# 0xC0000054/avif-format

Measured on NVIDIA H100. Metric: Gpixels/s, higher is better.
Workload: dtype f32

## Files before the change

### avif-format_b200/csrc/kernels_fast_flat.cu

```cuda
#include "kernels_fast_common.cuh"
#include "launch_keys.h"
#include "table_staging.cuh"
#include "../../include/avifgpu.h"

namespace avifgpu
{

using namespace avifpix;
using namespace fastenc;
using namespace staging;
using avifmath::LibmTables;

namespace
{

constexpr int kFlatThreads = kFlatWarps * 32;
constexpr int kRowSegmentBytes = kTilePixels * 12;
static_assert(kFlatStageBytesPerWarp == 2 * kRowSegmentBytes, "a warp's staging buffer holds both rows of its tile");
constexpr int kRowSegmentWords = kRowSegmentBytes / 4;
constexpr int kTableBarrierSlot = kFlatSharedBarriers / 8 - 1;
static_assert(kFlatWarps <= kTableBarrierSlot, "the warps' barriers and the table's share kFlatSharedBarriers");

struct FlatSchedule
{
    int32_t tilesX, tileRows, warpCount;
    int32_t segments, items;
    int32_t segmentRows, longSegments;
    int32_t lastColumnBytes;
    int32_t unpairedTileRow;
};

__device__ __forceinline__ bool ElectOne()
{
    uint32_t elected;
    asm volatile("{ .reg .pred p; elect.sync _|p, 0xffffffff; selp.u32 %0, 1, 0, p; }" : "=r"(elected));
    return elected != 0;
}

constexpr int kTableTwoLevel = 1;
constexpr int kTableCompact = 2;
constexpr int kTableCompact14 = 3;

template <int CURVE, int XS, int YS, int TABLE, int INTERLEAVED, int DEST>
__device__ __forceinline__ void EncodeRgbF32FlatBody(const FastEncodeParams& p, const FlatSchedule& schedule)
{
    constexpr bool kCompact = TABLE != kTableTwoLevel;
    constexpr int kCompactShift = TABLE == kTableCompact14 ? 14 : 0;
    extern __shared__ __align__(128) uint8_t sharedBytes[];
    uint64_t* libmStorage = reinterpret_cast<uint64_t*>(sharedBytes);
    uint64_t* barriers = reinterpret_cast<uint64_t*>(sharedBytes + kSharedLibm);
    uint8_t* stageAll = sharedBytes + kSharedLibm + kFlatSharedBarriers;
    uint32_t* compactEntries = reinterpret_cast<uint32_t*>(sharedBytes + FlatFixedBytes());
    const uint32_t* firstBits = compactEntries + ((p.table.flatCount + 3) & ~3);
    uint2* octaves = reinterpret_cast<uint2*>(sharedBytes + FlatFixedBytes());
    uint32_t* bucketWords = reinterpret_cast<uint32_t*>(sharedBytes + FlatFixedBytes() + kFlatOctaveBytes);

    const int lane = threadIdx.x & 31;
    const int warpInBlock = __shfl_sync(0xffffffffu, static_cast<int>(threadIdx.x >> 5), 0);
    const uint32_t barrier = SharedAddress(barriers + warpInBlock);
    uint32_t* stage = reinterpret_cast<uint32_t*>(stageAll + warpInBlock * kFlatStageBytesPerWarp);
    const uint32_t stageAddress = SharedAddress(stage);
    const uint32_t* myStage = stage + lane * 12;

    const int tilesX = schedule.tilesX;
    const int warpCount = schedule.warpCount;
    const int firstItem = warpInBlock * static_cast<int>(gridDim.x) + static_cast<int>(blockIdx.x);
    constexpr int kChromaRowsPerTile = YS ? 1 : 2;
    constexpr int kChromaPairs = SourceInterleaved(DEST) ? 2 : 1;
    constexpr int kChromaTileBytes = (XS ? kTilePixels : 2 * kTilePixels) * kChromaPairs;

    auto itemRows = [&](int item, int& column, int& rowBegin, int& rowEnd)
    {
        const int segment = item / tilesX;
        column = item - segment * tilesX;
        rowBegin = segment * schedule.segmentRows + min(segment, schedule.longSegments);
        rowEnd = rowBegin + schedule.segmentRows + (segment < schedule.longSegments ? 1 : 0);
    };
    auto fetchTile = [&](int row, uint32_t bytes, int64_t offset)
    {
        const bool second = row != schedule.unpairedTileRow;
        const uint8_t* source = p.rows + offset;
        BarrierExpect(barrier, second ? 2u * bytes : bytes);
        BulkCopyToShared(stageAddress, source, bytes, barrier);
        if (second)
        {
            BulkCopyToShared(stageAddress + kRowSegmentBytes, source + p.rowStride, bytes, barrier);
        }
    };
    auto columnBytes = [&](int column) { return column == tilesX - 1 ? static_cast<uint32_t>(schedule.lastColumnBytes) : static_cast<uint32_t>(kRowSegmentBytes); };
    auto sourceOffsetOf = [&](int row, int column) { return static_cast<int64_t>(row) * 2 * p.rowStride + static_cast<int64_t>(column) * kRowSegmentBytes; };

    if (kCompact && threadIdx.x == 0)
    {
        BeginTableImageCopy(p.table, compactEntries, barriers + kTableBarrierSlot);
    }
    if (ElectOne())
    {
        BarrierInit(barrier, 1);
        BarrierInitFence();
        if (firstItem < schedule.items)
        {
            int column, rowBegin, rowEnd;
            itemRows(firstItem, column, rowBegin, rowEnd);
            if (rowBegin < rowEnd)
            {
                fetchTile(rowBegin, columnBytes(column), sourceOffsetOf(rowBegin, column));
            }
        }
    }

    const LibmTables t = avifmath::StageLibmTables(libmStorage, threadIdx.x, blockDim.x);
    if (!kCompact)
    {
        for (int i = threadIdx.x; i < 256; i += blockDim.x)
        {
            octaves[i] = p.table.octaves[i];
        }
        for (int i = threadIdx.x; i < p.table.bucketCount; i += blockDim.x)
        {
            bucketWords[i] = p.table.buckets[i];
        }
    }
    __syncthreads();
    if (kCompact)
    {
        WaitTableImage(barriers + kTableBarrierSlot);
    }

    const uint32_t flatShift = p.table.flatShift;
    const int32_t negativeLow = -static_cast<int32_t>(p.table.flatLow);
    const int32_t span = static_cast<int32_t>(p.table.flatHigh - p.table.flatLow);
    const uint32_t bandStrideLog2 = p.table.bandStrideLog2;
    const uint32_t* __restrict__ bandBits = p.table.bandBits;
    const uint32_t compactTopShift = 32u - flatShift;
    const uint32_t compactCodeMask = p.table.compactCodeMask;
    const uint32_t compactMagic = p.table.compactMagic;
    uint32_t parity = 0;

#pragma unroll 1
    for (int item = firstItem; item < schedule.items; item += warpCount)
    {
        int column, rowBegin, rowEnd;
        itemRows(item, column, rowBegin, rowEnd);
        if (item != firstItem && rowBegin < rowEnd && ElectOne())
        {
            fetchTile(rowBegin, columnBytes(column), sourceOffsetOf(rowBegin, column));
        }
        const uint32_t tileBytes = columnBytes(column);
        const bool laneActive = column * kTilePixels + lane * 4 < p.width;
        int64_t sourceOffset = sourceOffsetOf(rowBegin, column);
        uint8_t* yPointer = p.planeY + static_cast<int64_t>(rowBegin) * 2 * p.strideY +
                            (INTERLEAVED ? static_cast<int64_t>(column) * (6 * kTilePixels) + lane * 24 : static_cast<int64_t>(column) * (2 * kTilePixels) + lane * 8);
        uint8_t* cbPointer = p.planeCb + static_cast<int64_t>(rowBegin) * kChromaRowsPerTile * p.strideCb + static_cast<int64_t>(column) * kChromaTileBytes + lane * (XS ? 4 : 8) * kChromaPairs;
        uint8_t* crPointer = p.planeCr + static_cast<int64_t>(rowBegin) * kChromaRowsPerTile * p.strideCr + static_cast<int64_t>(column) * kChromaTileBytes + lane * (XS ? 4 : 8);

#pragma unroll 1
    for (int tileRow = rowBegin; tileRow < rowEnd; ++tileRow)
    {
        const bool secondRow = tileRow != schedule.unpairedTileRow;
        sourceOffset += 2 * p.rowStride;

        BarrierWait(barrier, parity);
        parity ^= 1u;

        float codeF[kValuesPerLane];
        uint32_t bandMask = 0;
        int32_t largest = 0;
#pragma unroll
        for (int q = 0; q < 6; ++q)
        {
            const uint4 w = *reinterpret_cast<const uint4*>(myStage + (q / 3) * kRowSegmentWords + (q % 3) * 4);
            const uint32_t bits[4] = { w.x, w.y, w.z, w.w };
#pragma unroll
            for (int e = 0; e < 4; ++e)
            {
                const int j = 4 * q + e;
                bool inBand;
                if (kCompact)
                {
                    uint32_t entry;
                    codeF[j] = LookupCurveCompact<kCompactShift>(bits[e], compactEntries, flatShift, negativeLow, span, compactTopShift, compactCodeMask,
                                                                 compactMagic, inBand, entry);
                }
                else
                {
                    codeF[j] = CodeToFloat(LookupCurveCode(bits[e], octaves, bucketWords, inBand));
                }
                asm("{ .reg .pred p; setp.ne.u32 p, %1, 0; @p or.b32 %0, %0, %2; }" : "+r"(bandMask) : "r"(static_cast<uint32_t>(inBand)), "r"(1u << j));
            }
            if (kCompact)
            {
                largest = max(largest, __vimax3_s32(static_cast<int32_t>(w.x), static_cast<int32_t>(w.y), static_cast<int32_t>(w.z)));
                largest = max(largest, static_cast<int32_t>(w.w));
            }
        }

        auto stagedBits = [&](int j) { return myStage[j + (j >= 12 ? kRowSegmentWords - 12 : 0)]; };
        uint32_t lowerMask = 0;
        if (kCompact)
        {
            uint32_t pending = bandMask;
            while (pending != 0)
            {
                uint32_t word[2] = { 0xffffffffu, 0xffffffffu }, index[2] = { 0u, 0u }, sampleBit[2] = { 0u, 0u };
#pragma unroll
                for (int u = 0; u < 2; ++u)
                {
                    if (pending != 0)
                    {
                        const int j = __ffs(static_cast<int>(pending)) - 1;
                        pending &= pending - 1;
                        const uint32_t bits = stagedBits(j);
                        const int32_t bucket = __viaddmin_s32_relu(static_cast<int32_t>(bits) >> flatShift, negativeLow, span);
                        const uint32_t entry = compactEntries[bucket];
                        const uint32_t k = ((entry & compactCodeMask) >> kCompactLenBits) + ((entry >> compactTopShift) != 0 ? 1u : 0u);
                        const uint32_t distance = bits - firstBits[k];
                        if (k != 0 && distance < (1u << bandStrideLog2))
                        {
                            index[u] = (k << bandStrideLog2) + distance;
                            word[u] = __ldg(bandBits + (index[u] >> 5));
                            sampleBit[u] = 1u << j;
                        }
                    }
                }
#pragma unroll
                for (int u = 0; u < 2; ++u)
                {
                    if (((word[u] >> (index[u] & 31u)) & 1u) == 0)
                    {
                        lowerMask |= sampleBit[u];
                    }
                }
            }
        }

        if (__any_sync(0xffffffffu, kCompact ? largest > 0x7f7fffff : bandMask != 0))
        {
            for (int j = 0; j < kValuesPerLane; ++j)
            {
                const uint32_t bits = stagedBits(j);
                if (kCompact ? static_cast<int32_t>(bits) > 0x7f7fffff : ((bandMask >> j) & 1u) != 0)
                {
                    const float exact = CodeToFloat(ExactCurveCode<CURVE>(__uint_as_float(bits), p.pqMultiplier, p.maxCodeFloat, t));
#pragma unroll
                    for (int slot = 0; slot < kValuesPerLane; ++slot)
                    {
                        if (slot == j)
                        {
                            codeF[slot] = exact;
                        }
                    }
                }
            }
        }

        __syncwarp();
        if (tileRow + 1 < rowEnd && ElectOne())
        {
            fetchTile(tileRow + 1, tileBytes, sourceOffset);
        }

#pragma unroll
        for (int j = 0; j < kValuesPerLane; ++j)
        {
            if (lowerMask & (1u << j))
            {
                codeF[j] -= 1.0f;
            }
        }

        if (laneActive)
        {
            if (INTERLEAVED)
            {
#pragma unroll
                for (int r = 0; r < 2; ++r)
                {
                    if (r == 1 && !secondRow) break;
                    uint32_t words[6];
#pragma unroll
                    for (int w = 0; w < 6; ++w)
                    {
                        words[w] = __float2uint_rz(codeF[12 * r + 2 * w]) | (__float2uint_rz(codeF[12 * r + 2 * w + 1]) << 16);
                    }
                    uint2* target = reinterpret_cast<uint2*>(yPointer + r * p.strideY);
                    __stcs(target, make_uint2(words[0], words[1]));
                    __stcs(target + 1, make_uint2(words[2], words[3]));
                    __stcs(target + 2, make_uint2(words[4], words[5]));
                }
            }
            else
            {
                StoreTile<XS, YS, DEST>(p, codeF, yPointer, cbPointer, crPointer, secondRow);
            }
        }
        yPointer += 2 * p.strideY;
        cbPointer += kChromaRowsPerTile * p.strideCb;
        crPointer += kChromaRowsPerTile * p.strideCr;
    }
    }
}

template <int CURVE, int XS, int YS, int TABLE, int INTERLEAVED>
__global__ void __launch_bounds__(kFlatThreads, 1) EncodeRgbF32FlatKernel(const FastEncodeParams p, const FlatSchedule schedule)
{
    EncodeRgbF32FlatBody<CURVE, XS, YS, TABLE, INTERLEAVED, AVIFGPU_SOURCE_PLANAR>(p, schedule);
}

template <int CURVE, int XS, int YS, int TABLE, int DEST>
__global__ void __launch_bounds__(kFlatThreads, 1) EncodeDestRgbF32FlatKernel(const FastEncodeParams p, const FlatSchedule schedule)
{
    EncodeRgbF32FlatBody<CURVE, XS, YS, TABLE, 0, DEST>(p, schedule);
}

template <int CURVE, int XS, int YS, int TABLE, int INTERLEAVED, int DEST>
constexpr auto FlatKernelFor()
{
    if constexpr (DEST == AVIFGPU_SOURCE_PLANAR)
    {
        return EncodeRgbF32FlatKernel<CURVE, XS, YS, TABLE, INTERLEAVED>;
    }
    else
    {
        return EncodeDestRgbF32FlatKernel<CURVE, XS, YS, TABLE, DEST>;
    }
}

template <int CURVE, int XS, int YS, int TABLE, int INTERLEAVED = 0, int DEST = AVIFGPU_SOURCE_PLANAR>
cudaError_t LaunchFlatKernel(const FastEncodeParams& fp, int smCount, cudaStream_t stream)
{
    const size_t shared = static_cast<size_t>(FlatFixedBytes()) + FlatTableBytes(fp.table, TABLE == kTableTwoLevel);
    static std::atomic<uint64_t> configuredDevices{ 0 };
    {
        const cudaError_t e = AllowDynamicShared(FlatKernelFor<CURVE, XS, YS, TABLE, INTERLEAVED, DEST>(), kSharedLimit, configuredDevices);
        if (e != cudaSuccess)
        {
            return e;
        }
    }
    const long long tiles = static_cast<long long>((fp.width + kTilePixels - 1) / kTilePixels) * ((fp.rowCount + 1) / 2);
    if (tiles > 0x7fffffffll || shared > static_cast<size_t>(kSharedLimit))
    {
        return cudaErrorInvalidValue;
    }
    long long blocks = (tiles + kFlatWarps - 1) / kFlatWarps;
    if (blocks > smCount)
    {
        blocks = smCount;
    }
    FlatSchedule schedule{};
    schedule.tilesX = (fp.width + kTilePixels - 1) / kTilePixels;
    schedule.tileRows = (fp.rowCount + 1) / 2;
    schedule.warpCount = static_cast<int32_t>(blocks) * kFlatWarps;
    schedule.segments = schedule.warpCount / schedule.tilesX;
    if (schedule.segments < 1) schedule.segments = 1;
    if (schedule.segments > schedule.tileRows) schedule.segments = schedule.tileRows;
    schedule.items = schedule.tilesX * schedule.segments;
    schedule.segmentRows = schedule.tileRows / schedule.segments;
    schedule.longSegments = schedule.tileRows % schedule.segments;
    schedule.lastColumnBytes = (fp.width - (schedule.tilesX - 1) * kTilePixels) * 12;
    schedule.unpairedTileRow = (fp.rowCount & 1) ? fp.rowCount / 2 : -1;
    FlatKernelFor<CURVE, XS, YS, TABLE, INTERLEAVED, DEST>()<<<static_cast<unsigned>(blocks), kFlatThreads, shared, stream>>>(fp, schedule);
    return cudaGetLastError();
}

}

cudaError_t LaunchFastEncodeFlatInterleaved(const FastEncodeParams& fp, int curve, int smCount, cudaStream_t stream)
{
    if (FlatCompactFits(fp.table))
    {
        if (curve == kCurveLinearToPQ)
        {
            return fp.table.flatShift == 14 ? LaunchFlatKernel<kCurveLinearToPQ, 0, 0, kTableCompact14, 1>(fp, smCount, stream)
                                            : LaunchFlatKernel<kCurveLinearToPQ, 0, 0, kTableCompact, 1>(fp, smCount, stream);
        }
        return LaunchFlatKernel<kCurveLinearToSMPTE428, 0, 0, kTableCompact, 1>(fp, smCount, stream);
    }
    if (curve == kCurveLinearToPQ) return LaunchFlatKernel<kCurveLinearToPQ, 0, 0, kTableTwoLevel, 1>(fp, smCount, stream);
    return LaunchFlatKernel<kCurveLinearToSMPTE428, 0, 0, kTableTwoLevel, 1>(fp, smCount, stream);
}

cudaError_t LaunchFastEncodeFlat(const FastEncodeParams& fp, int curve, int xs, int ys, int dest, int smCount, cudaStream_t stream)
{
    return WithChroma(xs, ys, [&](auto XS, auto YS) {
        return WithLayout(dest, [&](auto DEST) {
            if (FlatCompactFits(fp.table))
            {
                if (curve == kCurveLinearToPQ)
                {
                    return fp.table.flatShift == 14 ? LaunchFlatKernel<kCurveLinearToPQ, XS(), YS(), kTableCompact14, 0, DEST()>(fp, smCount, stream)
                                                    : LaunchFlatKernel<kCurveLinearToPQ, XS(), YS(), kTableCompact, 0, DEST()>(fp, smCount, stream);
                }
                return LaunchFlatKernel<kCurveLinearToSMPTE428, XS(), YS(), kTableCompact, 0, DEST()>(fp, smCount, stream);
            }
            if constexpr (DEST() == AVIFGPU_SOURCE_PLANAR)
            {
                if (curve == kCurveLinearToPQ) return LaunchFlatKernel<kCurveLinearToPQ, XS(), YS(), kTableTwoLevel>(fp, smCount, stream);
            }
            else if (curve == kCurveLinearToPQ)
            {
                return cudaErrorInvalidValue;
            }
            return LaunchFlatKernel<kCurveLinearToSMPTE428, XS(), YS(), kTableTwoLevel, 0, DEST()>(fp, smCount, stream);
        });
    });
}

}
```

### avif-format_b200/csrc/table_staging.cuh

```cuda
#ifndef AVIFGPU_TABLE_STAGING_CUH
#define AVIFGPU_TABLE_STAGING_CUH

#include "curve_tables.h"

#include <stdint.h>

namespace avifgpu
{
namespace staging
{

constexpr uint32_t kTableCopyChunk = 16384;

__device__ __forceinline__ uint32_t SharedAddress(const void* pointer) { return static_cast<uint32_t>(__cvta_generic_to_shared(pointer)); }

__device__ __forceinline__ void BarrierInit(uint32_t barrier, uint32_t arrivals)
{
    asm volatile("mbarrier.init.shared::cta.b64 [%0], %1;" ::"r"(barrier), "r"(arrivals) : "memory");
}

__device__ __forceinline__ void BarrierInitFence() { asm volatile("fence.mbarrier_init.release.cluster;" ::: "memory"); }

__device__ __forceinline__ void BarrierExpect(uint32_t barrier, uint32_t bytes)
{
    asm volatile("mbarrier.arrive.expect_tx.shared::cta.b64 _, [%0], %1;" ::"r"(barrier), "r"(bytes) : "memory");
}

__device__ __forceinline__ void BulkCopyToShared(uint32_t target, const void* source, uint32_t bytes, uint32_t barrier)
{
    asm volatile("cp.async.bulk.shared::cluster.global.mbarrier::complete_tx::bytes [%0], [%1], %2, [%3];" ::"r"(target), "l"(source), "r"(bytes),
                 "r"(barrier)
                 : "memory");
}

__device__ __forceinline__ void BarrierWait(uint32_t barrier, uint32_t parity)
{
    asm volatile(
        "{\n"
        ".reg .pred done;\n"
        "WAIT_LOOP:\n"
        "mbarrier.try_wait.parity.shared::cta.b64 done, [%0], %1;\n"
        "@done bra WAIT_DONE;\n"
        "bra WAIT_LOOP;\n"
        "WAIT_DONE:\n"
        "}\n" ::"r"(barrier),
        "r"(parity)
        : "memory");
}

__device__ __forceinline__ void BeginTableImageCopy(const CurveTableView& table, void* sharedImage, uint64_t* barrierStorage)
{
    const uint32_t barrier = SharedAddress(barrierStorage);
    BarrierInit(barrier, 1);
    BarrierInitFence();
    const uint32_t imageBytes = table.compactImageBytes;
    BarrierExpect(barrier, imageBytes);
    const uint32_t target = SharedAddress(sharedImage);
    const uint8_t* source = reinterpret_cast<const uint8_t*>(table.compact);
    for (uint32_t offset = 0; offset < imageBytes; offset += kTableCopyChunk)
    {
        BulkCopyToShared(target + offset, source + offset, min(kTableCopyChunk, imageBytes - offset), barrier);
    }
}

__device__ __forceinline__ void WaitTableImage(uint64_t* barrierStorage) { BarrierWait(SharedAddress(barrierStorage), 0); }

}
}

#endif
```

Measured before the change: 184.8.

## Split tile fetch per row and prefetch second tile into L2

```diff
diff --git a/avif-format_b200/csrc/kernels_fast_flat.cu b/avif-format_b200/csrc/kernels_fast_flat.cu
--- a/avif-format_b200/csrc/kernels_fast_flat.cu
+++ b/avif-format_b200/csrc/kernels_fast_flat.cu
@@ -106,6 +106,15 @@
             {
                 fetchTile(rowBegin, columnBytes(column), sourceOffsetOf(rowBegin, column));
             }
+            if (rowBegin + 1 < rowEnd)
+            {
+                const uint8_t* second = p.rows + sourceOffsetOf(rowBegin + 1, column);
+                BulkPrefetchL2(second, columnBytes(column));
+                if (rowBegin + 1 != schedule.unpairedTileRow)
+                {
+                    BulkPrefetchL2(second + p.rowStride, columnBytes(column));
+                }
+            }
         }
     }
 
@@ -164,100 +173,116 @@
         parity ^= 1u;
 
         float codeF[kValuesPerLane];
-        uint32_t bandMask = 0;
-        int32_t largest = 0;
-#pragma unroll
-        for (int q = 0; q < 6; ++q)
-        {
-            const uint4 w = *reinterpret_cast<const uint4*>(myStage + (q / 3) * kRowSegmentWords + (q % 3) * 4);
-            const uint32_t bits[4] = { w.x, w.y, w.z, w.w };
-#pragma unroll
-            for (int e = 0; e < 4; ++e)
-            {
-                const int j = 4 * q + e;
-                bool inBand;
+        uint32_t lowerMask = 0;
+        const bool fetchNext = tileRow + 1 < rowEnd;
+        const bool nextSecondRow = tileRow + 1 != schedule.unpairedTileRow;
+#pragma unroll
+        for (int r = 0; r < 2; ++r)
+        {
+            const uint32_t* rowStage = myStage + r * kRowSegmentWords;
+
+            uint32_t bandMask = 0;
+            int32_t largest = 0;
+#pragma unroll
+            for (int q = 0; q < 3; ++q)
+            {
+                const uint4 w = *reinterpret_cast<const uint4*>(rowStage + q * 4);
+                const uint32_t bits[4] = { w.x, w.y, w.z, w.w };
+#pragma unroll
+                for (int e = 0; e < 4; ++e)
+                {
+                    const int j = 4 * q + e;
+                    bool inBand;
+                    if (kCompact)
+                    {
+                        uint32_t entry;
+                        codeF[12 * r + j] = LookupCurveCompact<kCompactShift>(bits[e], compactEntries, flatShift, negativeLow, span, compactTopShift,
+                                                                              compactCodeMask, compactMagic, inBand, entry);
+                    }
+                    else
+                    {
+                        codeF[12 * r + j] = CodeToFloat(LookupCurveCode(bits[e], octaves, bucketWords, inBand));
+                    }
+                    asm("{ .reg .pred p; setp.ne.u32 p, %1, 0; @p or.b32 %0, %0, %2; }" : "+r"(bandMask) : "r"(static_cast<uint32_t>(inBand)), "r"(1u << j));
+                }
                 if (kCompact)
                 {
-                    uint32_t entry;
-                    codeF[j] = LookupCurveCompact<kCompactShift>(bits[e], compactEntries, flatShift, negativeLow, span, compactTopShift, compactCodeMask,
-                                                                 compactMagic, inBand, entry);
+                    largest = max(largest, __vimax3_s32(static_cast<int32_t>(w.x), static_cast<int32_t>(w.y), static_cast<int32_t>(w.z)));
+                    largest = max(largest, static_cast<int32_t>(w.w));
+                }
+            }
+
+            if (kCompact)
+            {
+                uint32_t pending = bandMask;
+                while (pending != 0)
+                {
+                    uint32_t word[2] = { 0xffffffffu, 0xffffffffu }, index[2] = { 0u, 0u }, sampleBit[2] = { 0u, 0u };
+#pragma unroll
+                    for (int u = 0; u < 2; ++u)
+                    {
+                        if (pending != 0)
+                        {
+                            const int j = __ffs(static_cast<int>(pending)) - 1;
+                            pending &= pending - 1;
+                            const uint32_t bits = rowStage[j];
+                            const int32_t bucket = __viaddmin_s32_relu(static_cast<int32_t>(bits) >> flatShift, negativeLow, span);
+                            const uint32_t entry = compactEntries[bucket];
+                            const uint32_t k = ((entry & compactCodeMask) >> kCompactLenBits) + ((entry >> compactTopShift) != 0 ? 1u : 0u);
+                            const uint32_t distance = bits - firstBits[k];
+                            if (k != 0 && distance < (1u << bandStrideLog2))
+                            {
+                                index[u] = (k << bandStrideLog2) + distance;
+                                word[u] = __ldg(bandBits + (index[u] >> 5));
+                                sampleBit[u] = 1u << (12 * r + j);
+                            }
+                        }
+                    }
+#pragma unroll
+                    for (int u = 0; u < 2; ++u)
+                    {
+                        if (((word[u] >> (index[u] & 31u)) & 1u) == 0)
+                        {
+                            lowerMask |= sampleBit[u];
+                        }
+                    }
+                }
+            }
+
+            if (__any_sync(0xffffffffu, kCompact ? largest > 0x7f7fffff : bandMask != 0))
+            {
+                for (int j = 0; j < 12; ++j)
+                {
+                    const uint32_t bits = rowStage[j];
+                    if (kCompact ? static_cast<int32_t>(bits) > 0x7f7fffff : ((bandMask >> j) & 1u) != 0)
+                    {
+                        const float exact = CodeToFloat(ExactCurveCode<CURVE>(__uint_as_float(bits), p.pqMultiplier, p.maxCodeFloat, t));
+#pragma unroll
+                        for (int slot = 0; slot < 12; ++slot)
+                        {
+                            if (slot == j)
+                            {
+                                codeF[12 * r + slot] = exact;
+                            }
+                        }
+                    }
+                }
+            }
+
+            __syncwarp();
+            if (fetchNext && (r == 0 || nextSecondRow) && ElectOne())
+            {
+                const uint32_t half = stageAddress + r * kRowSegmentBytes;
+                if (r == 0 && nextSecondRow)
+                {
+                    BarrierExpectOnly(barrier, tileBytes);
                 }
                 else
                 {
-                    codeF[j] = CodeToFloat(LookupCurveCode(bits[e], octaves, bucketWords, inBand));
-                }
-                asm("{ .reg .pred p; setp.ne.u32 p, %1, 0; @p or.b32 %0, %0, %2; }" : "+r"(bandMask) : "r"(static_cast<uint32_t>(inBand)), "r"(1u << j));
-            }
-            if (kCompact)
-            {
-                largest = max(largest, __vimax3_s32(static_cast<int32_t>(w.x), static_cast<int32_t>(w.y), static_cast<int32_t>(w.z)));
-                largest = max(largest, static_cast<int32_t>(w.w));
-            }
-        }
-
-        auto stagedBits = [&](int j) { return myStage[j + (j >= 12 ? kRowSegmentWords - 12 : 0)]; };
-        uint32_t lowerMask = 0;
-        if (kCompact)
-        {
-            uint32_t pending = bandMask;
-            while (pending != 0)
-            {
-                uint32_t word[2] = { 0xffffffffu, 0xffffffffu }, index[2] = { 0u, 0u }, sampleBit[2] = { 0u, 0u };
-#pragma unroll
-                for (int u = 0; u < 2; ++u)
-                {
-                    if (pending != 0)
-                    {
-                        const int j = __ffs(static_cast<int>(pending)) - 1;
-                        pending &= pending - 1;
-                        const uint32_t bits = stagedBits(j);
-                        const int32_t bucket = __viaddmin_s32_relu(static_cast<int32_t>(bits) >> flatShift, negativeLow, span);
-                        const uint32_t entry = compactEntries[bucket];
-                        const uint32_t k = ((entry & compactCodeMask) >> kCompactLenBits) + ((entry >> compactTopShift) != 0 ? 1u : 0u);
-                        const uint32_t distance = bits - firstBits[k];
-                        if (k != 0 && distance < (1u << bandStrideLog2))
-                        {
-                            index[u] = (k << bandStrideLog2) + distance;
-                            word[u] = __ldg(bandBits + (index[u] >> 5));
-                            sampleBit[u] = 1u << j;
-                        }
-                    }
-                }
-#pragma unroll
-                for (int u = 0; u < 2; ++u)
-                {
-                    if (((word[u] >> (index[u] & 31u)) & 1u) == 0)
-                    {
-                        lowerMask |= sampleBit[u];
-                    }
-                }
-            }
-        }
-
-        if (__any_sync(0xffffffffu, kCompact ? largest > 0x7f7fffff : bandMask != 0))
-        {
-            for (int j = 0; j < kValuesPerLane; ++j)
-            {
-                const uint32_t bits = stagedBits(j);
-                if (kCompact ? static_cast<int32_t>(bits) > 0x7f7fffff : ((bandMask >> j) & 1u) != 0)
-                {
-                    const float exact = CodeToFloat(ExactCurveCode<CURVE>(__uint_as_float(bits), p.pqMultiplier, p.maxCodeFloat, t));
-#pragma unroll
-                    for (int slot = 0; slot < kValuesPerLane; ++slot)
-                    {
-                        if (slot == j)
-                        {
-                            codeF[slot] = exact;
-                        }
-                    }
-                }
-            }
-        }
-
-        __syncwarp();
-        if (tileRow + 1 < rowEnd && ElectOne())
-        {
-            fetchTile(tileRow + 1, tileBytes, sourceOffset);
+                    BarrierExpect(barrier, tileBytes);
+                }
+                BulkCopyToShared(half, p.rows + sourceOffset + r * p.rowStride, tileBytes, barrier);
+            }
         }
 
 #pragma unroll
diff --git a/avif-format_b200/csrc/table_staging.cuh b/avif-format_b200/csrc/table_staging.cuh
--- a/avif-format_b200/csrc/table_staging.cuh
+++ b/avif-format_b200/csrc/table_staging.cuh
@@ -26,11 +26,21 @@
     asm volatile("mbarrier.arrive.expect_tx.shared::cta.b64 _, [%0], %1;" ::"r"(barrier), "r"(bytes) : "memory");
 }
 
+__device__ __forceinline__ void BarrierExpectOnly(uint32_t barrier, uint32_t bytes)
+{
+    asm volatile("mbarrier.expect_tx.relaxed.cta.shared::cta.b64 [%0], %1;" ::"r"(barrier), "r"(bytes) : "memory");
+}
+
 __device__ __forceinline__ void BulkCopyToShared(uint32_t target, const void* source, uint32_t bytes, uint32_t barrier)
 {
     asm volatile("cp.async.bulk.shared::cluster.global.mbarrier::complete_tx::bytes [%0], [%1], %2, [%3];" ::"r"(target), "l"(source), "r"(bytes),
                  "r"(barrier)
                  : "memory");
+}
+
+__device__ __forceinline__ void BulkPrefetchL2(const void* source, uint32_t bytes)
+{
+    asm volatile("cp.async.bulk.prefetch.L2.global [%0], %1;" ::"l"(source), "r"(bytes) : "memory");
 }
 
 __device__ __forceinline__ void BarrierWait(uint32_t barrier, uint32_t parity)
diff --git a/profiles/measure_flat_rounds.py b/profiles/measure_flat_rounds.py
--- /dev/null
+++ b/profiles/measure_flat_rounds.py
@@ -0,0 +1,78 @@
+#!/usr/bin/env python3
+import statistics
+import subprocess
+
+import harness
+import numpy as np
+import torch
+
+import avifgpu
+import bench
+
+HEIGHTS = (1080, 2160, 4320, 8640)
+FLAT_WARPS = 28
+TILE_PIXELS = 128
+
+
+def tiles_per_warp(width, height, sms):
+    tiles_x, tile_rows = (width + TILE_PIXELS - 1) // TILE_PIXELS, (height + 1) // 2
+    blocks = min(sms, (tiles_x * tile_rows + FLAT_WARPS - 1) // FLAT_WARPS)
+    segments = min(max(blocks * FLAT_WARPS // tiles_x, 1), tile_rows)
+    return tile_rows / segments
+
+
+def sm_clock_mhz():
+    try:
+        out = subprocess.run(["nvidia-smi", "--query-gpu=clocks.sm", "--format=csv,noheader,nounits", "-i", "0"],
+                             capture_output=True, text=True, timeout=10).stdout
+        return float(out.strip().splitlines()[0])
+    except Exception:
+        return None
+
+
+def main():
+    args = harness.arguments(rounds=5).parse_args()
+    harness.require_gpu()
+    sms = torch.cuda.get_device_properties(0).multi_processor_count
+    device = torch.device("cuda", 0)
+    with avifgpu.Context(0) as ctx:
+        runs, ways = {}, {}
+        for h in HEIGHTS:
+            run = runs[h] = bench.DeviceRun(torch, avifgpu, ctx, bench.Workload("c2", rows=h), device, 2000 + h)
+            step = [0]
+
+            def call(run=run, step=step):
+                run.launch(step[0])
+                step[0] += 1
+
+            ways[h] = call
+        before = ctx.launch_count()
+        ways[HEIGHTS[0]]()
+        torch.cuda.synchronize()
+        launches = ctx.launch_count() - before
+        times = harness.timed(ways, args.seconds, args.rounds)
+        clock = sm_clock_mhz()
+
+    points = {}
+    for h in HEIGHTS:
+        us = [ms * 1e3 for ms in times[h]]
+        points[h] = {"bytes": runs[h].wl.algorithmic_bytes, "median_us": statistics.median(us), "spread_us": max(us) - min(us),
+                     "tiles_per_warp": tiles_per_warp(runs[h].wl.w, h, sms)}
+    x = np.array([points[h]["bytes"] for h in HEIGHTS], dtype=np.float64)
+    y = np.array([points[h]["median_us"] for h in HEIGHTS], dtype=np.float64)
+    slope, fixed = np.polyfit(x, y, 1)
+    for h in HEIGHTS:
+        points[h]["fit_residual_us"] = points[h]["median_us"] - (fixed + slope * points[h]["bytes"])
+    frame = points[4320]
+    round_us = (frame["median_us"] - fixed) / frame["tiles_per_warp"]
+    result = {
+        "card": harness.card() | {"sm_mhz_after": clock}, "sms": sms, "launches_per_call": launches,
+        "fixed_us": fixed, "rate_tbs": 1.0 / slope / 1e6, "round_us": round_us, "fixed_rounds": fixed / round_us,
+        "points": {str(h): p for h, p in points.items()},
+        "unit": "microseconds per call (device events, median of rounds)",
+    }
+    harness.emit([result], args.out)
+
+
+if __name__ == "__main__":
+    main()
```

After: 184.8, median of 6. About the same (-0.0%).
